# modelscope/FunASR

Hardware: AMD Instinct MI355X
Metric: audio-seconds/sec (RTF^-1) Paraformer-large 30s@bs64 (higher is better)
Workload: dtype f32 (GEMM / self-attention operands split into 2 fp16 planes, 3 fp16 MFMA products, f32 accumulate; all else f32)

## Files before the change

### funasr_amd/csrc/attention_f16x2.hip

```cpp
#include "common.h"

namespace pf {

namespace {

constexpr int DK = 128, KT = 32;
constexpr int KP_B = KT * DK * 2;
constexpr int VP_B = DK * KT * 2;
constexpr int STAGE_B = 2 * KP_B + 2 * VP_B;
constexpr int OLD = DK + 4;
constexpr int SLAB_B = 8 * 32 * OLD * 4;
constexpr int LDS_BYTES = SLAB_B > 3 * STAGE_B ? SLAB_B : 3 * STAGE_B;
constexpr float P_SCALE = 1024.f;
typedef _Float16 f16x8 __attribute__((ext_vector_type(8)));

constexpr float LAZY_TAU = 3.0f;
template <int PIPE, bool LAZY = false>
__global__ __launch_bounds__(512, 2) void attention_f16x2_kernel(Attn2Args p) {
    extern __shared__ __attribute__((aligned(16))) unsigned char smem[];
    constexpr int NSTAGE = PIPE ? 3 : 2;
    constexpr int QB = 256;
    constexpr int NV = 1;

    const int tid = threadIdx.x, lane = tid & 63;
    const int wave = __builtin_amdgcn_readfirstlane(tid >> 6);
    const int hh = lane >> 5, idx = lane & 31;
    int b, head, qblk;
    if (p.xcd_nqb > 0) {
        const int L = blockIdx.x, j = L >> 3;
        const int pair = (j / p.xcd_nqb) * 8 + (L & 7);
        if (pair >= p.B * p.H) return;
        qblk = j % p.xcd_nqb; head = pair % p.H; b = pair / p.H;
    } else {
        b = blockIdx.z; head = blockIdx.y; qblk = blockIdx.x;
    }
    const int Tq = p.qoffs ? p.qoffs[b + 1] - p.qoffs[b] : (p.Tq > 0 ? p.Tq : p.Tp);
    if (qblk * QB >= Tq) return;
    const int q = qblk * QB + wave * 32 + idx;
    const int qc = q < Tq ? q : Tq - 1;
    const int klen = p.klens[b];
    const int kstart = p.koffs ? p.koffs[b] : b * p.Tp;
    const size_t row0 = (size_t)(kstart & ~15);
    const int kskip = kstart & 15, kend = kskip + klen;
    const size_t qrow0 = p.qoffs ? (size_t)p.qoffs[b] : (size_t)b * Tq;

    f16x8 qf[2][8];
    {
        const unsigned short* qp = p.Q + (qrow0 + qc) * p.ldq + head * DK + hh * 8;
#pragma unroll
        for (int pl = 0; pl < 2; ++pl)
#pragma unroll
            for (int s = 0; s < 8; ++s)
                qf[pl][s] = __builtin_bit_cast(f16x8, *reinterpret_cast<const uint4*>(qp + pl * p.q_plane + 16 * s));
    }

    floatx16 o[4];
#pragma unroll
    for (int d = 0; d < 4; ++d)
#pragma unroll
        for (int r = 0; r < 16; ++r) o[d][r] = 0.f;
    float m_run = -INFINITY, l_run = 0.f;

    const unsigned short* ksrc[NV];
    const unsigned short* vsrc[NV];
    unsigned lds_w[NV];
#pragma unroll
    for (int v = 0; v < NV; ++v) {
        const int vw = wave * NV + v;
        const int kr = vw * 4 + (lane >> 4);
        ksrc[v] = p.K + (row0 + kr) * p.ldk + head * DK + (((lane & 15) ^ (kr & 15)) * 8);
        const int dr = vw * 16 + (lane >> 2);
        vsrc[v] = p.VT + (size_t)(head * DK + dr) * p.ldvt + row0 + (((lane & 3) ^ ((dr >> 2) & 3)) * 8);
        lds_w[v] = __builtin_amdgcn_readfirstlane(lds_addr_of(smem) + (unsigned)vw * 1024);
    }
    auto stage = [&](int kt) {
        const size_t ko = (size_t)kt * KT * p.ldk;
#pragma unroll
        for (int v = 0; v < NV; ++v) {
            const unsigned base = lds_w[v] + (unsigned)(kt % NSTAGE) * STAGE_B;
            glds16(ksrc[v] + ko, base);
            glds16(ksrc[v] + p.k_plane + ko, base + KP_B);
            glds16(vsrc[v] + kt * KT, base + 2 * KP_B);
            glds16(vsrc[v] + p.vt_plane + kt * KT, base + 2 * KP_B + VP_B);
        }
    };

    const float sscale = p.sscale_dev ? p.sscale * *p.sscale_dev : p.sscale;
    const float sscale2 = LAZY ? sscale * 1.4426950408889634f : sscale;
#define PF_EXP(x_) (LAZY ? __builtin_amdgcn_exp2f(x_) : __expf(x_))
    constexpr float PSC = LAZY ? 1.f : P_SCALE;
    const int ntiles = (kend + KT - 1) / KT;

#define PF_QK(KT_, SA, SB)                                                                                            \
    {                                                                                                                 \
        const unsigned char* kp = smem + ((KT_) % NSTAGE) * STAGE_B + idx * 256;                                      \
        _Pragma("unroll") for (int r = 0; r < 16; ++r) { SA[r] = 0.f; SB[r] = 0.f; }                                  \
        _Pragma("unroll") for (int st = 0; st < 8; ++st) {                                                            \
            const int co = ((2 * st + hh) ^ (idx & 15)) * 16;                                                         \
            const f16x8 kh = __builtin_bit_cast(f16x8, *reinterpret_cast<const uint4*>(kp + co));                     \
            const f16x8 kl = __builtin_bit_cast(f16x8, *reinterpret_cast<const uint4*>(kp + KP_B + co));              \
            SA = __builtin_amdgcn_mfma_f32_32x32x16_f16(kl, qf[0][st], SA, 0, 0, 0);                                  \
            SB = __builtin_amdgcn_mfma_f32_32x32x16_f16(kh, qf[0][st], SB, 0, 0, 0);                                  \
            SA = __builtin_amdgcn_mfma_f32_32x32x16_f16(kh, qf[1][st], SA, 0, 0, 0);                                  \
        }                                                                                                             \
    }
#define PF_SOFTMAX(K0_, SA, SB)                                                                                       \
    {                                                                                                                 \
        float mx = -INFINITY;                                                                                         \
        if (LAZY && (K0_) >= kskip && (K0_) + KT <= kend) {         \
            _Pragma("unroll") for (int r = 0; r < 16; ++r) {                                                          \
                s[r] = (SA[r] + SB[r]) * sscale2;                                                                     \
                mx = fmaxf(mx, s[r]);                                                                                 \
            }                                                                                                         \
        } else {                                                                                                      \
            _Pragma("unroll") for (int r = 0; r < 16; ++r) {                                                          \
                const int key = (K0_) + (r & 3) + 8 * (r >> 2) + 4 * hh;                                              \
                s[r] = (unsigned)(key - kskip) < (unsigned)klen ? (SA[r] + SB[r]) * sscale2 : -INFINITY;              \
                mx = fmaxf(mx, s[r]);                                                                                 \
            }                                                                                                         \
        }                                                                                                             \
        mx = fmaxf(mx, __shfl_xor(mx, 32, 64));                                                                       \
        float m_new = fmaxf(m_run, mx);                                                                               \
        bool moved = true;                                                                                            \
        if constexpr (LAZY) {                         \
            moved = m_new > m_run + LAZY_TAU * 1.4426950408889634f;                                                                         \
            m_new = moved ? m_new : m_run;                                                                            \
        }                                                                                                             \
        const float alpha = moved ? PF_EXP(m_run - m_new) : 1.f;                                                      \
        float psum = 0.f;                                                                                             \
        const float m_off = LAZY ? m_new - 10.f : m_new;          \
        _Pragma("unroll") for (int r = 0; r < 16; ++r) {                                                              \
            s[r] = PF_EXP(s[r] - m_off);                                                                              \
            psum += s[r];                                                                                             \
        }                                                                                                             \
        psum += __shfl_xor(psum, 32, 64);                                                                             \
        l_run = l_run * alpha + psum;                                                                                 \
        m_run = m_new;                                                                                                \
        if (!LAZY || __any(moved)) {                                                                                  \
            _Pragma("unroll") for (int d = 0; d < 4; ++d) _Pragma("unroll") for (int r = 0; r < 16; ++r) o[d][r] *= alpha; \
        }                                                                                                             \
    }
#define PF_PV(KT_)                                                                                                    \
    {                                                                                                                 \
        const unsigned char* vp = smem + ((KT_) % NSTAGE) * STAGE_B + 2 * KP_B + idx * 64;                            \
        _Pragma("unroll") for (int st = 0; st < 2; ++st) {                                                            \
            uint4 ph, pl;                                                                                             \
            split2_pk(s[8 * st + 0] * PSC, s[8 * st + 1] * PSC, ph.x, pl.x);                                  \
            split2_pk(s[8 * st + 2] * PSC, s[8 * st + 3] * PSC, ph.y, pl.y);                                  \
            split2_pk(s[8 * st + 4] * PSC, s[8 * st + 5] * PSC, ph.z, pl.z);                                  \
            split2_pk(s[8 * st + 6] * PSC, s[8 * st + 7] * PSC, ph.w, pl.w);                                  \
            const f16x8 Ph = __builtin_bit_cast(f16x8, ph), Pl = __builtin_bit_cast(f16x8, pl);                       \
            const int co = ((2 * st + hh) ^ ((idx >> 2) & 3)) * 16;                                                   \
            f16x8 vf[4][2];                                                                                           \
            _Pragma("unroll") for (int d = 0; d < 4; ++d) _Pragma("unroll") for (int pn = 0; pn < 2; ++pn)            \
                vf[d][pn] = __builtin_bit_cast(f16x8, *reinterpret_cast<const uint4*>(vp + pn * VP_B + d * 32 * 64 + co)); \
            _Pragma("unroll") for (int d = 0; d < 4; ++d) o[d] = __builtin_amdgcn_mfma_f32_32x32x16_f16(vf[d][1], Ph, o[d], 0, 0, 0); \
            _Pragma("unroll") for (int d = 0; d < 4; ++d) o[d] = __builtin_amdgcn_mfma_f32_32x32x16_f16(vf[d][0], Pl, o[d], 0, 0, 0); \
            _Pragma("unroll") for (int d = 0; d < 4; ++d) o[d] = __builtin_amdgcn_mfma_f32_32x32x16_f16(vf[d][0], Ph, o[d], 0, 0, 0); \
        }                                                                                                             \
    }

    float s[16];
    const bool active = qblk * QB + wave * 32 < Tq;
    if constexpr (PIPE == 0) {
        stage(0);
        for (int kt = 0; kt < ntiles; ++kt) {
            glds_wait_all();
            __syncthreads();
            if (kt + 1 < ntiles) stage(kt + 1);
            if (active) {
                floatx16 sa, sb;
                PF_QK(kt, sa, sb)
                PF_SOFTMAX(kt * KT, sa, sb)
                PF_PV(kt)
            }
        }
    } else {
        floatx16 ca, cb, na, nb;
        stage(0);
        if (ntiles > 1) stage(1);
        glds_wait_all();
        __syncthreads();
        PF_QK(0, ca, cb)
        for (int kt = 0; kt < ntiles; ++kt) {
            if (kt > 0) { glds_wait_all(); __syncthreads(); }
            if (kt + 2 < ntiles) stage(kt + 2);
            const int kn = kt + 1 < ntiles ? kt + 1 : kt;
            PF_QK(kn, na, nb)
            PF_SOFTMAX(kt * KT, ca, cb)
#pragma unroll
            for (int g = 0; g < 24; ++g) {
                __builtin_amdgcn_sched_group_barrier(0x008, 1, 0);
                __builtin_amdgcn_sched_group_barrier(0x002, 7, 0);
            }
            PF_PV(kt)
            ca = na; cb = nb;
        }
    }
#undef PF_QK
#undef PF_EXP
#undef PF_SOFTMAX
#undef PF_PV

    __syncthreads();
    float* slab = reinterpret_cast<float*>(smem) + wave * (32 * OLD);
    {
        const float inv = (LAZY ? p.oscale * P_SCALE : p.oscale) / l_run;
#pragma unroll
        for (int d = 0; d < 4; ++d)
#pragma unroll
            for (int g = 0; g < 4; ++g) {
                const float4 t = make_float4(o[d][4 * g + 0] * inv, o[d][4 * g + 1] * inv, o[d][4 * g + 2] * inv, o[d][4 * g + 3] * inv);
                *reinterpret_cast<float4*>(slab + idx * OLD + d * 32 + 8 * g + 4 * hh) = t;
            }
    }
    const int qw0 = qblk * QB + wave * 32;
#pragma unroll
    for (int it = 0; it < 8; ++it) {
        const int rr = it * 4 + (lane >> 4), c8 = (lane & 15) * 8;
        const float4 a = *reinterpret_cast<const float4*>(slab + rr * OLD + c8);
        const float4 c = *reinterpret_cast<const float4*>(slab + rr * OLD + c8 + 4);
        if (qw0 + rr < Tq) {
            uint4 h, l;
            split2_pk(a.x, a.y, h.x, l.x);
            split2_pk(a.z, a.w, h.y, l.y);
            split2_pk(c.x, c.y, h.z, l.z);
            split2_pk(c.z, c.w, h.w, l.w);
            unsigned short* op = p.O + (qrow0 + qw0 + rr) * p.ldo + head * DK + c8;
            *reinterpret_cast<uint4*>(op) = h;
            *reinterpret_cast<uint4*>(op + p.o_plane) = l;
        }
    }
}

}

int launch_attention_f16x2(const Attn2Args& a, hipStream_t stream) {
    PF_REQUIRE(a.B > 0 && a.H > 0 && (a.koffs || (a.Tp > 0 && a.Tp % 16 == 0)), "attention_f16x2: rows per sequence must be a positive multiple of 16");
    PF_REQUIRE(a.ldq % 8 == 0 && a.ldk % 8 == 0 && a.ldvt % 8 == 0 && a.ldo % 8 == 0 && a.q_plane % 8 == 0 &&
               a.k_plane % 8 == 0 && a.vt_plane % 8 == 0 && a.o_plane % 8 == 0, "attention_f16x2: strides % 8");
    PF_REQUIRE(((uintptr_t)a.Q & 15) == 0 && ((uintptr_t)a.K & 15) == 0 && ((uintptr_t)a.VT & 15) == 0 && ((uintptr_t)a.O & 15) == 0,
               "attention_f16x2: 16-B alignment");
    static PerDeviceOnce configured;
    if (!configured.done()) {
#if defined(PF_MEASUREMENT_KERNELS)
        PF_HIP_TRY(hipFuncSetAttribute(reinterpret_cast<const void*>(&attention_f16x2_kernel<0>),
                                       hipFuncAttributeMaxDynamicSharedMemorySize, LDS_BYTES));
        PF_HIP_TRY(hipFuncSetAttribute(reinterpret_cast<const void*>(&attention_f16x2_kernel<1>),
                                       hipFuncAttributeMaxDynamicSharedMemorySize, LDS_BYTES));
#endif
        PF_HIP_TRY(hipFuncSetAttribute(reinterpret_cast<const void*>(&attention_f16x2_kernel<0, true>),
                                       hipFuncAttributeMaxDynamicSharedMemorySize, LDS_BYTES));
        configured.mark();
    }
    const int rows = a.Tq > 0 ? a.Tq : a.Tp;
    Attn2Args k = a;
#if defined(PF_MEASUREMENT_KERNELS)
    PF_REQUIRE(a.variant == 0 || a.variant == 1 || a.variant == 3, "attention_f16x2: variant must be 0, 1 or 3");
#else
    PF_REQUIRE(a.variant == 3, "attention_f16x2: variant must be 3 (variants 0 / 1: the measurement library, make measure)");
#endif
    const int nqb = ceil_div(rows, 256);
    dim3 grid(nqb, a.H, a.B);
    k.xcd_nqb = (a.xcd_nqb >= 0 && nqb > 1) ? nqb : 0;
    if (k.xcd_nqb > 0) grid = dim3((unsigned)(ceil_div(a.B * a.H, 8) * 8 * nqb), 1, 1);
    if (a.variant == 3)
        hipLaunchKernelGGL((attention_f16x2_kernel<0, true>), grid, dim3(512), LDS_BYTES, stream, k);
#if defined(PF_MEASUREMENT_KERNELS)
    else if (a.variant == 1)
        hipLaunchKernelGGL(attention_f16x2_kernel<1>, grid, dim3(512), LDS_BYTES, stream, k);
    else
        hipLaunchKernelGGL(attention_f16x2_kernel<0>, grid, dim3(512), LDS_BYTES, stream, k);
#endif
    PF_HIP_TRY(hipGetLastError());
    return 0;
}

}
```

Baseline: 40550.

## Switch attention kernel from 32x32x16 to 16x16x32 MFMA tiles

Moves the split-fp16 attention kernel from 32x32x16 MFMA tiles to 16x16x32 tiles. Each wave now covers two 16-query blocks and two 16-key blocks, and the K/V LDS swizzles and fragment addressing are reworked to match. The softmax row max and sum now reduce across four lane groups using permlane swap builtins, and the scheduling barriers are regrouped. The goal is better MFMA throughput or latency and fewer LDS bank conflicts, in exchange for more reduction shuffles and a more complex swizzle that must stay consistent between the staging and read paths.

Measured after the change: 41130, median of 6. 1.4% higher.

```diff
diff --git a/funasr_amd/csrc/attention_f16x2.hip b/funasr_amd/csrc/attention_f16x2.hip
--- a/funasr_amd/csrc/attention_f16x2.hip
+++ b/funasr_amd/csrc/attention_f16x2.hip
@@ -13,6 +13,20 @@
 constexpr int LDS_BYTES = SLAB_B > 3 * STAGE_B ? SLAB_B : 3 * STAGE_B;
 constexpr float P_SCALE = 1024.f;
 typedef _Float16 f16x8 __attribute__((ext_vector_type(8)));
+struct ScoreTiles { floatx4 t[2][2]; };
+
+__device__ __forceinline__ float quad_max(float x) {
+    auto r = __builtin_amdgcn_permlane32_swap(__float_as_uint(x), __float_as_uint(x), false, false);
+    x = fmaxf(__uint_as_float(r[0]), __uint_as_float(r[1]));
+    r = __builtin_amdgcn_permlane16_swap(__float_as_uint(x), __float_as_uint(x), false, false);
+    return fmaxf(__uint_as_float(r[0]), __uint_as_float(r[1]));
+}
+__device__ __forceinline__ float quad_sum(float x) {
+    auto r = __builtin_amdgcn_permlane32_swap(__float_as_uint(x), __float_as_uint(x), false, false);
+    x = __uint_as_float(r[0]) + __uint_as_float(r[1]);
+    r = __builtin_amdgcn_permlane16_swap(__float_as_uint(x), __float_as_uint(x), false, false);
+    return __uint_as_float(r[0]) + __uint_as_float(r[1]);
+}
 
 constexpr float LAZY_TAU = 3.0f;
 template <int PIPE, bool LAZY = false>
@@ -24,7 +38,7 @@
 
     const int tid = threadIdx.x, lane = tid & 63;
     const int wave = __builtin_amdgcn_readfirstlane(tid >> 6);
-    const int hh = lane >> 5, idx = lane & 31;
+    const int g = lane >> 4, col = lane & 15;
     int b, head, qblk;
     if (p.xcd_nqb > 0) {
         const int L = blockIdx.x, j = L >> 3;
@@ -36,30 +50,33 @@
     }
     const int Tq = p.qoffs ? p.qoffs[b + 1] - p.qoffs[b] : (p.Tq > 0 ? p.Tq : p.Tp);
     if (qblk * QB >= Tq) return;
-    const int q = qblk * QB + wave * 32 + idx;
-    const int qc = q < Tq ? q : Tq - 1;
     const int klen = p.klens[b];
     const int kstart = p.koffs ? p.koffs[b] : b * p.Tp;
     const size_t row0 = (size_t)(kstart & ~15);
     const int kskip = kstart & 15, kend = kskip + klen;
     const size_t qrow0 = p.qoffs ? (size_t)p.qoffs[b] : (size_t)b * Tq;
 
-    f16x8 qf[2][8];
-    {
-        const unsigned short* qp = p.Q + (qrow0 + qc) * p.ldq + head * DK + hh * 8;
+    f16x8 qf[2][2][4];
+#pragma unroll
+    for (int qb = 0; qb < 2; ++qb) {
+        const int q = qblk * QB + wave * 32 + qb * 16 + col;
+        const int qc = q < Tq ? q : Tq - 1;
+        const unsigned short* qp = p.Q + (qrow0 + qc) * p.ldq + head * DK + g * 8;
 #pragma unroll
         for (int pl = 0; pl < 2; ++pl)
 #pragma unroll
-            for (int s = 0; s < 8; ++s)
-                qf[pl][s] = __builtin_bit_cast(f16x8, *reinterpret_cast<const uint4*>(qp + pl * p.q_plane + 16 * s));
-    }
-
-    floatx16 o[4];
-#pragma unroll
-    for (int d = 0; d < 4; ++d)
-#pragma unroll
-        for (int r = 0; r < 16; ++r) o[d][r] = 0.f;
-    float m_run = -INFINITY, l_run = 0.f;
+            for (int s = 0; s < 4; ++s)
+                qf[pl][qb][s] = __builtin_bit_cast(f16x8, *reinterpret_cast<const uint4*>(qp + pl * p.q_plane + 32 * s));
+    }
+
+    floatx4 o[8][2];
+#pragma unroll
+    for (int d = 0; d < 8; ++d)
+#pragma unroll
+        for (int qb = 0; qb < 2; ++qb)
+#pragma unroll
+            for (int r = 0; r < 4; ++r) o[d][qb][r] = 0.f;
+    float m_run[2] = {-INFINITY, -INFINITY}, l_run[2] = {0.f, 0.f};
 
     const unsigned short* ksrc[NV];
     const unsigned short* vsrc[NV];
@@ -68,9 +85,9 @@
     for (int v = 0; v < NV; ++v) {
         const int vw = wave * NV + v;
         const int kr = vw * 4 + (lane >> 4);
-        ksrc[v] = p.K + (row0 + kr) * p.ldk + head * DK + (((lane & 15) ^ (kr & 15)) * 8);
+        ksrc[v] = p.K + (row0 + kr) * p.ldk + head * DK + (((lane & 15) ^ ((kr & 7) | ((kr >> 1) & 8))) * 8);
         const int dr = vw * 16 + (lane >> 2);
-        vsrc[v] = p.VT + (size_t)(head * DK + dr) * p.ldvt + row0 + (((lane & 3) ^ ((dr >> 2) & 3)) * 8);
+        vsrc[v] = p.VT + (size_t)(head * DK + dr) * p.ldvt + row0 + (((lane & 3) ^ (-(dr >> 2) & 3)) * 8);
         lds_w[v] = __builtin_amdgcn_readfirstlane(lds_addr_of(smem) + (unsigned)vw * 1024);
     }
     auto stage = [&](int kt) {
@@ -91,94 +108,127 @@
     constexpr float PSC = LAZY ? 1.f : P_SCALE;
     const int ntiles = (kend + KT - 1) / KT;
 
+    const int arow = 16 * (col >> 3) + (col & 7);
+    const int kbase = 16 * (g >> 1) + 4 * (g & 1);
 #define PF_QK(KT_, SA, SB)                                                                                            \
     {                                                                                                                 \
-        const unsigned char* kp = smem + ((KT_) % NSTAGE) * STAGE_B + idx * 256;                                      \
-        _Pragma("unroll") for (int r = 0; r < 16; ++r) { SA[r] = 0.f; SB[r] = 0.f; }                                  \
-        _Pragma("unroll") for (int st = 0; st < 8; ++st) {                                                            \
-            const int co = ((2 * st + hh) ^ (idx & 15)) * 16;                                                         \
-            const f16x8 kh = __builtin_bit_cast(f16x8, *reinterpret_cast<const uint4*>(kp + co));                     \
-            const f16x8 kl = __builtin_bit_cast(f16x8, *reinterpret_cast<const uint4*>(kp + KP_B + co));              \
-            SA = __builtin_amdgcn_mfma_f32_32x32x16_f16(kl, qf[0][st], SA, 0, 0, 0);                                  \
-            SB = __builtin_amdgcn_mfma_f32_32x32x16_f16(kh, qf[0][st], SB, 0, 0, 0);                                  \
-            SA = __builtin_amdgcn_mfma_f32_32x32x16_f16(kh, qf[1][st], SA, 0, 0, 0);                                  \
+        const unsigned char* kp = smem + ((KT_) % NSTAGE) * STAGE_B + arow * 256;                                     \
+        _Pragma("unroll") for (int kb = 0; kb < 2; ++kb) _Pragma("unroll") for (int qb = 0; qb < 2; ++qb)             \
+            _Pragma("unroll") for (int r = 0; r < 4; ++r) { SA.t[kb][qb][r] = 0.f; SB.t[kb][qb][r] = 0.f; }           \
+        _Pragma("unroll") for (int st = 0; st < 4; ++st) {                                                            \
+            const int co = ((4 * st + g) ^ col) * 16;                                                                 \
+            f16x8 kh[2], kl[2];                                                                                       \
+            _Pragma("unroll") for (int kb = 0; kb < 2; ++kb) {                                                        \
+                kh[kb] = __builtin_bit_cast(f16x8, *reinterpret_cast<const uint4*>(kp + kb * 8 * 256 + co));          \
+                kl[kb] = __builtin_bit_cast(f16x8, *reinterpret_cast<const uint4*>(kp + KP_B + kb * 8 * 256 + co));   \
+            }                                                                                                         \
+            _Pragma("unroll") for (int kb = 0; kb < 2; ++kb) _Pragma("unroll") for (int qb = 0; qb < 2; ++qb)         \
+                SA.t[kb][qb] = __builtin_amdgcn_mfma_f32_16x16x32_f16(kl[kb], qf[0][qb][st], SA.t[kb][qb], 0, 0, 0);  \
+            _Pragma("unroll") for (int kb = 0; kb < 2; ++kb) _Pragma("unroll") for (int qb = 0; qb < 2; ++qb)         \
+                SB.t[kb][qb] = __builtin_amdgcn_mfma_f32_16x16x32_f16(kh[kb], qf[0][qb][st], SB.t[kb][qb], 0, 0, 0);  \
+            _Pragma("unroll") for (int kb = 0; kb < 2; ++kb) _Pragma("unroll") for (int qb = 0; qb < 2; ++qb)         \
+                SA.t[kb][qb] = __builtin_amdgcn_mfma_f32_16x16x32_f16(kh[kb], qf[1][qb][st], SA.t[kb][qb], 0, 0, 0);  \
         }                                                                                                             \
     }
 #define PF_SOFTMAX(K0_, SA, SB)                                                                                       \
     {                                                                                                                 \
-        float mx = -INFINITY;                                                                                         \
+        float mx[2] = {-INFINITY, -INFINITY};                                                                         \
         if (LAZY && (K0_) >= kskip && (K0_) + KT <= kend) {         \
-            _Pragma("unroll") for (int r = 0; r < 16; ++r) {                                                          \
-                s[r] = (SA[r] + SB[r]) * sscale2;                                                                     \
-                mx = fmaxf(mx, s[r]);                                                                                 \
+            _Pragma("unroll") for (int qb = 0; qb < 2; ++qb) _Pragma("unroll") for (int kb = 0; kb < 2; ++kb)         \
+                _Pragma("unroll") for (int r = 0; r < 4; ++r) {                                                       \
+                    const float x = (SA.t[kb][qb][r] + SB.t[kb][qb][r]) * sscale2;                                    \
+                    s[8 * qb + 4 * kb + r] = x;                                                                       \
+                    mx[qb] = fmaxf(mx[qb], x);                                                                        \
+                }                                                                                                     \
+        } else {                                                                                                      \
+            _Pragma("unroll") for (int qb = 0; qb < 2; ++qb) _Pragma("unroll") for (int kb = 0; kb < 2; ++kb)         \
+                _Pragma("unroll") for (int r = 0; r < 4; ++r) {                                                       \
+                    const int key = (K0_) + kbase + 8 * kb + r;                                                       \
+                    const float x = (unsigned)(key - kskip) < (unsigned)klen ? (SA.t[kb][qb][r] + SB.t[kb][qb][r]) * sscale2 : -INFINITY; \
+                    s[8 * qb + 4 * kb + r] = x;                                                                       \
+                    mx[qb] = fmaxf(mx[qb], x);                                                                        \
+                }                                                                                                     \
+        }                                                                                                             \
+        float alpha[2];                                                                                               \
+        bool moved_any = false;                                                                                       \
+        _Pragma("unroll") for (int qb = 0; qb < 2; ++qb) {                                                            \
+            float m_new = fmaxf(m_run[qb], quad_max(mx[qb]));                                                         \
+            bool moved = true;                                                                                        \
+            if constexpr (LAZY) {                     \
+                moved = m_new > m_run[qb] + LAZY_TAU * 1.4426950408889634f;                                           \
+                m_new = moved ? m_new : m_run[qb];                                                                    \
             }                                                                                                         \
-        } else {                                                                                                      \
-            _Pragma("unroll") for (int r = 0; r < 16; ++r) {                                                          \
-                const int key = (K0_) + (r & 3) + 8 * (r >> 2) + 4 * hh;                                              \
-                s[r] = (unsigned)(key - kskip) < (unsigned)klen ? (SA[r] + SB[r]) * sscale2 : -INFINITY;              \
-                mx = fmaxf(mx, s[r]);                                                                                 \
+            alpha[qb] = moved ? PF_EXP(m_run[qb] - m_new) : 1.f;                                                      \
+            float psum = 0.f;                                                                                         \
+            const float m_off = LAZY ? m_new - 10.f : m_new;      \
+            _Pragma("unroll") for (int r = 0; r < 8; ++r) {                                                           \
+                s[8 * qb + r] = PF_EXP(s[8 * qb + r] - m_off);                                                        \
+                psum += s[8 * qb + r];                                                                                \
             }                                                                                                         \
-        }                                                                                                             \
-        mx = fmaxf(mx, __shfl_xor(mx, 32, 64));                                                                       \
-        float m_new = fmaxf(m_run, mx);                                                                               \
-        bool moved = true;                                                                                            \
-        if constexpr (LAZY) {                         \
-            moved = m_new > m_run + LAZY_TAU * 1.4426950408889634f;                                                                         \
-            m_new = moved ? m_new : m_run;                                                                            \
-        }                                                                                                             \
-        const float alpha = moved ? PF_EXP(m_run - m_new) : 1.f;                                                      \
-        float psum = 0.f;                                                                                             \
-        const float m_off = LAZY ? m_new - 10.f : m_new;          \
-        _Pragma("unroll") for (int r = 0; r < 16; ++r) {                                                              \
-            s[r] = PF_EXP(s[r] - m_off);                                                                              \
-            psum += s[r];                                                                                             \
-        }                                                                                                             \
-        psum += __shfl_xor(psum, 32, 64);                                                                             \
-        l_run = l_run * alpha + psum;                                                                                 \
-        m_run = m_new;                                                                                                \
-        if (!LAZY || __any(moved)) {                                                                                  \
-            _Pragma("unroll") for (int d = 0; d < 4; ++d) _Pragma("unroll") for (int r = 0; r < 16; ++r) o[d][r] *= alpha; \
+            l_run[qb] = l_run[qb] * alpha[qb] + quad_sum(psum);                                                       \
+            m_run[qb] = m_new;                                                                                        \
+            moved_any = moved_any || moved;                                                                           \
+        }                                                                                                             \
+        if (!LAZY || __any(moved_any)) {                                                                              \
+            _Pragma("unroll") for (int d = 0; d < 8; ++d) _Pragma("unroll") for (int qb = 0; qb < 2; ++qb)            \
+                _Pragma("unroll") for (int r = 0; r < 4; ++r) o[d][qb][r] *= alpha[qb];                               \
         }                                                                                                             \
     }
 #define PF_PV(KT_)                                                                                                    \
     {                                                                                                                 \
-        const unsigned char* vp = smem + ((KT_) % NSTAGE) * STAGE_B + 2 * KP_B + idx * 64;                            \
-        _Pragma("unroll") for (int st = 0; st < 2; ++st) {                                                            \
+        const unsigned char* vp = smem + ((KT_) % NSTAGE) * STAGE_B + 2 * KP_B + col * 64 + ((g ^ (-(col >> 2) & 3)) * 16); \
+        f16x8 Ph[2], Pl[2];                                                                                           \
+        _Pragma("unroll") for (int qb = 0; qb < 2; ++qb) {                                                            \
             uint4 ph, pl;                                                                                             \
-            split2_pk(s[8 * st + 0] * PSC, s[8 * st + 1] * PSC, ph.x, pl.x);                                  \
-            split2_pk(s[8 * st + 2] * PSC, s[8 * st + 3] * PSC, ph.y, pl.y);                                  \
-            split2_pk(s[8 * st + 4] * PSC, s[8 * st + 5] * PSC, ph.z, pl.z);                                  \
-            split2_pk(s[8 * st + 6] * PSC, s[8 * st + 7] * PSC, ph.w, pl.w);                                  \
-            const f16x8 Ph = __builtin_bit_cast(f16x8, ph), Pl = __builtin_bit_cast(f16x8, pl);                       \
-            const int co = ((2 * st + hh) ^ ((idx >> 2) & 3)) * 16;                                                   \
+            split2_pk(s[8 * qb + 0] * PSC, s[8 * qb + 1] * PSC, ph.x, pl.x);                                          \
+            split2_pk(s[8 * qb + 2] * PSC, s[8 * qb + 3] * PSC, ph.y, pl.y);                                          \
+            split2_pk(s[8 * qb + 4] * PSC, s[8 * qb + 5] * PSC, ph.z, pl.z);                                          \
+            split2_pk(s[8 * qb + 6] * PSC, s[8 * qb + 7] * PSC, ph.w, pl.w);                                          \
+            Ph[qb] = __builtin_bit_cast(f16x8, ph); Pl[qb] = __builtin_bit_cast(f16x8, pl);                           \
+        }                                                                                                             \
+        _Pragma("unroll") for (int dh = 0; dh < 8; dh += 4) {                                                         \
             f16x8 vf[4][2];                                                                                           \
             _Pragma("unroll") for (int d = 0; d < 4; ++d) _Pragma("unroll") for (int pn = 0; pn < 2; ++pn)            \
-                vf[d][pn] = __builtin_bit_cast(f16x8, *reinterpret_cast<const uint4*>(vp + pn * VP_B + d * 32 * 64 + co)); \
-            _Pragma("unroll") for (int d = 0; d < 4; ++d) o[d] = __builtin_amdgcn_mfma_f32_32x32x16_f16(vf[d][1], Ph, o[d], 0, 0, 0); \
-            _Pragma("unroll") for (int d = 0; d < 4; ++d) o[d] = __builtin_amdgcn_mfma_f32_32x32x16_f16(vf[d][0], Pl, o[d], 0, 0, 0); \
-            _Pragma("unroll") for (int d = 0; d < 4; ++d) o[d] = __builtin_amdgcn_mfma_f32_32x32x16_f16(vf[d][0], Ph, o[d], 0, 0, 0); \
-        }                                                                                                             \
-    }
+                vf[d][pn] = __builtin_bit_cast(f16x8, *reinterpret_cast<const uint4*>(vp + pn * VP_B + (dh + d) * 16 * 64)); \
+            _Pragma("unroll") for (int d = 0; d < 4; ++d) _Pragma("unroll") for (int qb = 0; qb < 2; ++qb)            \
+                o[dh + d][qb] = __builtin_amdgcn_mfma_f32_16x16x32_f16(vf[d][1], Ph[qb], o[dh + d][qb], 0, 0, 0);     \
+            _Pragma("unroll") for (int d = 0; d < 4; ++d) _Pragma("unroll") for (int qb = 0; qb < 2; ++qb)            \
+                o[dh + d][qb] = __builtin_amdgcn_mfma_f32_16x16x32_f16(vf[d][0], Pl[qb], o[dh + d][qb], 0, 0, 0);     \
+            _Pragma("unroll") for (int d = 0; d < 4; ++d) _Pragma("unroll") for (int qb = 0; qb < 2; ++qb)            \
+                o[dh + d][qb] = __builtin_amdgcn_mfma_f32_16x16x32_f16(vf[d][0], Ph[qb], o[dh + d][qb], 0, 0, 0);     \
+        }                                                                                                             \
+    }
+
+    auto q_loaded = [&]() {
+#pragma unroll
+        for (int pl = 0; pl < 2; ++pl)
+#pragma unroll
+            for (int qb = 0; qb < 2; ++qb)
+#pragma unroll
+                for (int st = 0; st < 4; ++st) asm volatile("" : "+v"(qf[pl][qb][st]));
+    };
 
     float s[16];
     const bool active = qblk * QB + wave * 32 < Tq;
     if constexpr (PIPE == 0) {
         stage(0);
+        q_loaded();
         for (int kt = 0; kt < ntiles; ++kt) {
             glds_wait_all();
             __syncthreads();
             if (kt + 1 < ntiles) stage(kt + 1);
             if (active) {
-                floatx16 sa, sb;
+                ScoreTiles sa, sb;
                 PF_QK(kt, sa, sb)
                 PF_SOFTMAX(kt * KT, sa, sb)
                 PF_PV(kt)
             }
         }
     } else {
-        floatx16 ca, cb, na, nb;
+        ScoreTiles ca, cb, na, nb;
         stage(0);
         if (ntiles > 1) stage(1);
+        q_loaded();
         glds_wait_all();
         __syncthreads();
         PF_QK(0, ca, cb)
@@ -189,9 +239,9 @@
             PF_QK(kn, na, nb)
             PF_SOFTMAX(kt * KT, ca, cb)
 #pragma unroll
-            for (int g = 0; g < 24; ++g) {
+            for (int i = 0; i < 48; ++i) {
                 __builtin_amdgcn_sched_group_barrier(0x008, 1, 0);
-                __builtin_amdgcn_sched_group_barrier(0x002, 7, 0);
+                __builtin_amdgcn_sched_group_barrier(0x002, 4, 0);
             }
             PF_PV(kt)
             ca = na; cb = nb;
@@ -204,15 +254,14 @@
 
     __syncthreads();
     float* slab = reinterpret_cast<float*>(smem) + wave * (32 * OLD);
-    {
-        const float inv = (LAZY ? p.oscale * P_SCALE : p.oscale) / l_run;
-#pragma unroll
-        for (int d = 0; d < 4; ++d)
-#pragma unroll
-            for (int g = 0; g < 4; ++g) {
-                const float4 t = make_float4(o[d][4 * g + 0] * inv, o[d][4 * g + 1] * inv, o[d][4 * g + 2] * inv, o[d][4 * g + 3] * inv);
-                *reinterpret_cast<float4*>(slab + idx * OLD + d * 32 + 8 * g + 4 * hh) = t;
-            }
+#pragma unroll
+    for (int qb = 0; qb < 2; ++qb) {
+        const float inv = (LAZY ? p.oscale * P_SCALE : p.oscale) / l_run[qb];
+#pragma unroll
+        for (int d = 0; d < 8; ++d) {
+            const float4 t = make_float4(o[d][qb][0] * inv, o[d][qb][1] * inv, o[d][qb][2] * inv, o[d][qb][3] * inv);
+            *reinterpret_cast<float4*>(slab + (qb * 16 + col) * OLD + d * 16 + 4 * g) = t;
+        }
     }
     const int qw0 = qblk * QB + wave * 32;
 #pragma unroll
```
